# uber/aresdb

Hardware: AMD Instinct MI355X
Metric: rows/sec, 1B-row filter -> group-by-agg (whole job) (higher is better)
Workload: dtype u32 keys / f64 sums; 1 GPU; C3: filter d1<90 -> dims [floor(ts,3600), d1, d2, d3] (4 x uint32) -> SUM(m float32 -> float64) via HashReduce, validity bitmaps with 1% nulls, shard resident in HBM; rows_per_gpu=1000000000, batch_rows=67108864, batches=15, streams_per_query=2, parallelism=1 shard(s), one per GPU

## Files before the change

### aresdb_amd/abi.py

```python
import ctypes as C
import os

_HERE = os.path.dirname(os.path.abspath(__file__))
REPO_ROOT = os.path.dirname(_HERE)
LIB_DIR = os.environ.get("ARES_LIB_DIR") or os.path.join(_HERE, "lib")

AGGR_SUM_UNSIGNED, AGGR_SUM_SIGNED, AGGR_SUM_FLOAT = 1, 2, 3
AGGR_MIN_UNSIGNED, AGGR_MIN_SIGNED, AGGR_MIN_FLOAT = 4, 5, 6
AGGR_MAX_UNSIGNED, AGGR_MAX_SIGNED, AGGR_MAX_FLOAT = 7, 8, 9
AGGR_HLL, AGGR_AVG_FLOAT = 10, 11

(Bool, Int8, Uint8, Int16, Uint16, Int32, Uint32, Float32, Int64, Uint64, Float64, GeoPoint,
 UUID) = range(13)
ConstInt, ConstFloat, ConstGeoPoint, ConstUUID = range(4)
(Negate, Not, BitwiseNot, IsNull, IsNotNull, Noop, GetWeekStart, GetMonthStart, GetQuarterStart,
 GetYearStart, GetDayOfMonth, GetDayOfYear, GetMonthOfYear, GetQuarterOfYear, GetHLLValue,
 ArrayLength) = range(16)
(And, Or, Equal, NotEqual, LessThan, LessThanOrEqual, GreaterThan, GreaterThanOrEqual, Plus, Minus,
 Multiply, Divide, Mod, BitwiseAnd, BitwiseOr, BitwiseXor, Floor, ArrayContains,
 ArrayElementAt) = range(19)
(VectorPartyInput, ScratchSpaceInput, ConstantInput, ForeignColumnInput,
 ArrayVectorPartyInput) = range(5)
ScratchSpaceOutput, MeasureOutput, DimensionOutput = range(3)
NUM_DIM_WIDTH = 5
# ... 277 lines not shown
    def hint_fused_batch(self, query, batch_rows, prev_size, measure_bytes, stream=None, device=0):
        fn = self._algo.AresHintFusedBatch
        fn.argtypes, fn.restype = [C.POINTER(FusedQuery), C.c_int, C.c_int, C.c_int, _S, _I], None
        fn(C.byref(query), int(batch_rows), int(prev_size), int(measure_bytes), stream, device)

    SCAN_AT_FILTER_COUNTERS = ("hints", "scans", "honoured", "declined", "discard_plan", "discard_shape", "discard_touched",
                               "discard_abandoned", "retried", "latched")

    def scan_at_filter_stats(self):
        c = (C.c_ulonglong * len(self.SCAN_AT_FILTER_COUNTERS))()
        self._algo.AresScanAtFilterStats.argtypes, self._algo.AresScanAtFilterStats.restype = [C.POINTER(C.c_ulonglong)], None
        self._algo.AresScanAtFilterStats(c)
        return {k: int(v) for k, v in zip(self.SCAN_AT_FILTER_COUNTERS, c)}

    @property
    def has_fused_select(self):
        return hasattr(self._algo, "AresFusedFilterSelect")

    def fused_filter_select(self, query, batch_rows, limit, out_keys, stream=None, device=0):
        fn = self._algo.AresFusedFilterSelect
        fn.argtypes = [C.POINTER(FusedSelect), C.c_int, C.c_int, DimensionVector, _S, _I]
        fn.restype = CGoCallResHandle
        return _check(fn(C.byref(query), int(batch_rows), int(limit), out_keys, stream, device))

    def select_stats(self):
        c = (C.c_ulonglong * 4)()
        self._algo.AresSelectStats.argtypes, self._algo.AresSelectStats.restype = [C.POINTER(C.c_ulonglong)], None
        self._algo.AresSelectStats(c)
        return {"batches": int(c[0]), "declined": int(c[1]), "tiles": int(c[2]), "rows": int(c[3])}

# ... 128 lines not shown
```

### aresdb_amd/csrc/algo/fused_consumers.hip

```cpp
#include <hip/hip_runtime.h>

#include <cstring>
#include <string>

#include "ares_extensions.h"

#include "deferral.hpp"
#include "hash_reduce_lds.hpp"
#include "sort_reduce_fused.hpp"

namespace ares {

namespace {
struct QueueMatch {
  int prev = 0;
  int dimJob[kFusedDims], measureJob = -1;
  const FilterJournal *journal = nullptr;
  int n0 = 0;
};
bool match_queue(const PendingQueue &pq, const DimensionVector &in, const DimLayoutD &L, int length, QueueMatch *m) {
  const int nd = L.numDims, prev = m->prev = length - pq.n;
  const size_t cap = static_cast<size_t>(in.VectorCapacity);
  if (pq.n <= 0 || prev < 0 || nd < 1 || nd > kFusedDims || in.NumDimsPerDimWidth[0] || in.NumDimsPerDimWidth[1]) return false;
  if (pq.jobs.count != nd && pq.jobs.count != nd + 1) return false;
// ... 131 lines not shown
  *groups = result;
  return true;
}

namespace {
bool hinted_operands(const AresFusedExpr &e, bool compareOnly, int batchRows, hipStream_t stream, FastOperands &f) {
  if (e.arity != 1 && e.arity != 2) return false;
  if (e.lhs.Type != VectorPartyInput || (e.arity == 2 && e.rhs.Type != ConstantInput)) return false;
  if (static_cast<int64_t>(e.lhs.Vector.VP.Length) < batchRows) return false;
  InputVector ins[2] = {e.lhs, e.arity == 2 ? e.rhs : e.lhs};
  EvalParams p;
  CallTemps temps;
  build_params(ins, e.arity, stream, nullptr, nullptr, 0, e.functor, p, temps);
  return p.a.length >= static_cast<uint32_t>(batchRows) && fast_operands(p, f, compareOnly) && f.step == 4;
}
bool hint_fused_batch(int device, hipStream_t stream, const AresFusedQuery &q, int batchRows, int prevSize, int measureBytes) {
  if (!fuse_available() || !row_space_enabled() || !scan_at_filter_enabled()) return false;
  if (q.numDims < 1 || q.numDims > kGenericFusedDims || q.numFilters < 1 || q.numFilters > kExtensionFilters) return false;
  if (batchRows <= 0 || prevSize < 0 || static_cast<int64_t>(batchRows) + prevSize > INT32_MAX) return false;
  if (measureBytes != 4 && measureBytes != 8) return false;
  const int mt = q.measure.outType;
  if (!(mt == Int32 || mt == Uint32 || mt == Float32 || mt == Int64 || mt == Float64) || measureBytes != ((mt == Int64 || mt == Float64) ? 8 : 4))
    return false;
  AggSpec a;
  if (!supported_agg_spec(q.aggFunc, measureBytes, hash_reduce_lds_supported, &a)) return false;
  ScanHint h;
  memset(&h, 0, sizeof(h));
  const int nd = q.numDims;
  h.nd = nd;
  h.batchRows = batchRows;
  h.prevSize = prevSize;
  auto note = [&](const FastOperands &f) {
    column_ranges(f, static_cast<uint32_t>(batchRows), [&](const ByteRange &c) { h.ranges[h.numRanges++] = ScanHint::Range{c.lo, c.hi}; });
  };
  SinkD sink;
  FastOperands f;
  for (int d = 0; d < nd; d++) {
    const int t = q.dims[d].outType;
    if (!(t == Int32 || t == Uint32 || t == Float32) || !hinted_operands(q.dims[d], false, batchRows, stream, f)) return false;
    memset(&sink, 0, sizeof(sink));
    sink.type = SINK_DIM;
// ... 7 lines not shown
  sink.type = SINK_MEASURE;
  sink.dtype = mt;
  sink.width = measureBytes;
  sink.agg = q.aggFunc;
  sink.identity = identity_bits(q.aggFunc, mt);
  if (sink.agg == AGGR_AVG_FLOAT || (measureBytes == 8 && sink.identity != 0)) return false;
  fused_plan_measure(h.plan, nd, f, sink, measureBytes);
  note(f);
  for (int k = 0; k < q.numFilters; k++) {
    if (!hinted_operands(q.filters[k], true, batchRows, stream, f)) return false;
    f.idx = nullptr;
    h.filters[k] = f;
    note(f);
  }
  if (!fused_plan_filters(h.plan, h.filters, static_cast<size_t>(q.numFilters))) return false;
  if (h.plan.numCols > nd + 2 || fused_plan_narrow(h.plan, nd)) return false;
  scan_hint_set(device, stream, h);
  return true;
}
}

namespace {
bool same_vector(const DimensionVector &a, const DimensionVector &b) {
  return a.DimValues == b.DimValues && a.HashValues == b.HashValues && a.IndexVector == b.IndexVector && a.VectorCapacity == b.VectorCapacity &&
         memcmp(a.NumDimsPerDimWidth, b.NumDimsPerDimWidth, sizeof(a.NumDimsPerDimWidth)) == 0;
}
}

static void mark_sort_output(const PendingSort &ps, void *at, size_t bytes, int unit) {
  uint8_t *p = static_cast<uint8_t *>(at);
  retire_fills(range_of(p, bytes), false);
  t_state->fills[p] = PendingFill{ps.stream, bytes, 0, unit, false, ps.keys.IndexVector};
}
// ... 246 lines not shown

void AresHintFusedBatch(const AresFusedQuery *query, int batchRows, int prevSize, int measureBytes, void *cudaStream, int device) {
  bool taken = false;
  try {
    taken = query != nullptr && device >= 0 && device < kMaxDevices &&
            hint_fused_batch(device, reinterpret_cast<hipStream_t>(cudaStream), *query, batchRows, prevSize, measureBytes);
  } catch (std::exception &) {
  }
  if (!taken) scan_ahead_count(kScanAheadDeclined);
}

void AresScanAtFilterStats(unsigned long long *counters) {
  if (counters) scan_ahead_stats(counters);
}

}
```

### aresdb_amd/csrc/algo/hash_reduce_lds.hip

```cpp
#include <hip/hip_runtime.h>

#include <atomic>
#include <functional>
#include <map>
#include <mutex>
#include <string>
#include <unordered_map>

#include <memory>
#include <mutex>
#include <vector>

#include "aggregate.hpp"
#include "common.hpp"
#include "device_model.hpp"
#include "ares_extensions.h"
#include "dim_layout.hpp"
#include "fast_eval.hpp"
#include "hash_reduce_lds.hpp"
#include "hr_kernels.hpp"
#include "hr_rtc.hpp"
#include "sort_reduce_fused.hpp"

namespace ares {
// ... 569 lines not shown
}
static void prepare_direct_scan(Regions &r, const FusedPlanD &plan, int partBits, int64_t rowsA, int batchRows, int prevSize, int streams,
                                int chunkTiles, hipStream_t stream) {
  SlowScope slow("make_regions");
  make_regions(r, partBits, rowsA, batchRows, streams, 4, stream, chunkTiles > 0 ? static_cast<int>(kCompactLineRecords) : 8);
  r.ws.widen = widen_of(plan);
  r.ws.chunkRows = static_cast<uint32_t>(chunkTiles) * 4096u;
  r.ws.rowBase = static_cast<uint32_t>(prevSize);
}

struct ScanStash {
  Regions r;
  FusedPlanD plan;
  int nd, batchRows, prevSize, partBits, chunkTiles, slack;
  RtcKernel lean;
};
namespace {
struct AheadEntry {
  int device;
  hipStream_t stream;
  bool live = false;
  int inits = 0;
  ScanHint hint;
  std::shared_ptr<ScanStash> stash;
  int discardsInARow = 0;
  bool latched = false;
  FusedPlanD latchedShape;
};
std::mutex g_aheadMutex;
std::vector<AheadEntry> g_ahead;
std::atomic<unsigned long long> g_aheadCounters[kScanAheadCounters];

AheadEntry *ahead_find(int device, hipStream_t stream) {
  for (AheadEntry &e : g_ahead)
    if (e.device == device && e.stream == stream) return &e;
  return nullptr;
}
FusedPlanD shape_of(FusedPlanD plan) {
  for (int c = 0; c < kFusedCols; c++) {
    plan.cols[c].vals = nullptr;
    plan.cols[c].nulls = nullptr;
    plan.cols[c].bitOff = 0;
  }
  return plan;
}
void ahead_discarded(AheadEntry &e, int reason) {
  scan_ahead_count(reason);
  if (reason == kScanAheadDiscardRetry) return;
  if (++e.discardsInARow >= 2 && !e.latched) {
    e.latched = true;
    e.latchedShape = shape_of(e.hint.plan);
  }
}
bool ranges_hit(const ScanHint &h, const uint8_t *lo, const uint8_t *hi) {
  for (int k = 0; k < h.numRanges; k++)
    if (h.ranges[k].lo < hi && lo < h.ranges[k].hi) return true;
  return false;
}
}

void scan_ahead_count(int which) { g_aheadCounters[which].fetch_add(1, std::memory_order_relaxed); }
void scan_ahead_stats(unsigned long long *out) {
  for (int k = 0; k < kScanAheadCounters; k++) out[k] = g_aheadCounters[k].load(std::memory_order_relaxed);
}
bool scan_at_filter_enabled() {
  static EnvSwitch<bool> on("ARES_SCAN_AT_FILTER", [](const char *e) { return !(e && e[0] == '0'); });
  return on.get() && grouped_enabled();
}

void scan_hint_set(int device, hipStream_t stream, const ScanHint &hint) {
  std::shared_ptr<ScanStash> old;
  {
    std::lock_guard<std::mutex> lock(g_aheadMutex);
    AheadEntry *e = ahead_find(device, stream);
    if (!e) {
      g_ahead.emplace_back();
      e = &g_ahead.back();
      e->device = device;
      e->stream = stream;
    }
    if (e->stash) ahead_discarded(*e, kScanAheadDiscardAbandoned);
    old.swap(e->stash);
    if (e->latched && fused_plan_equal(shape_of(hint.plan), e->latchedShape, hint.nd)) {
      scan_ahead_count(kScanAheadLatched);
      e->live = false;
      return;
    }
    if (e->latched) {
      e->latched = false;
      e->discardsInARow = 0;
    }
    e->hint = hint;
    e->live = true;
    e->inits = 0;
    scan_ahead_count(kScanAheadHints);
  }
}

void scan_hint_init_index(int device, hipStream_t stream) {
  std::shared_ptr<ScanStash> old;
  std::lock_guard<std::mutex> lock(g_aheadMutex);
  AheadEntry *e = ahead_find(device, stream);
  if (!e) return;
  if (e->stash) ahead_discarded(*e, kScanAheadDiscardAbandoned);
  old.swap(e->stash);
  if (e->live && ++e->inits > 1) e->live = false;
}

bool scan_hint_live(int device, hipStream_t stream, ScanHint *out) {
  std::lock_guard<std::mutex> lock(g_aheadMutex);
  AheadEntry *e = ahead_find(device, stream);
  if (!e || !e->live || e->inits != 1 || e->stash) return false;
  *out = e->hint;
  return true;
}

void scan_stash_put(int device, hipStream_t stream, std::shared_ptr<ScanStash> stash) {
  std::lock_guard<std::mutex> lock(g_aheadMutex);
  AheadEntry *e = ahead_find(device, stream);
  if (!e || !e->live) return;
// ... 17 lines not shown
  if (reason == kScanAheadHonoured) {
    scan_ahead_count(kScanAheadHonoured);
    if (e) e->discardsInARow = 0;
  } else if (e && blame) {
    ahead_discarded(*e, reason);
  } else {
    scan_ahead_count(reason);
  }
}

void scan_ahead_note_touch(int device, const void *ptr, size_t bytes, bool freed) {
  const uint8_t *lo = static_cast<const uint8_t *>(ptr), *hi = lo + (bytes ? bytes : 1);
  std::vector<std::shared_ptr<ScanStash>> dead;
  std::lock_guard<std::mutex> lock(g_aheadMutex);
  for (AheadEntry &e : g_ahead) {
    if (e.device != device || !(e.live || e.stash) || !ranges_hit(e.hint, lo, hi)) continue;
    e.live = false;
    if (e.stash && !freed) {
      scan_ahead_count(kScanAheadDiscardTouched);
      dead.push_back(std::move(e.stash));
      e.stash = nullptr;
    }
  }
}

void scan_ahead_stream_gone(int device, hipStream_t stream) {
  std::shared_ptr<ScanStash> old;
  std::lock_guard<std::mutex> lock(g_aheadMutex);
  for (size_t i = 0; i < g_ahead.size(); i++)
    if (g_ahead[i].device == device && g_ahead[i].stream == stream) {
      if (g_ahead[i].stash) scan_ahead_count(kScanAheadDiscardAbandoned);
      old.swap(g_ahead[i].stash);
      g_ahead[i] = g_ahead.back();
      g_ahead.pop_back();
      return;
    }
}

std::shared_ptr<ScanStash> fused_scan_ahead(int device, const ScanHint &hint, hipStream_t stream, uint32_t *hostCount, int *grid) {
  const FusedPlanD &plan = hint.plan;
  const bool narrow = fused_plan_narrow(plan, hint.nd);
  const int64_t length = static_cast<int64_t>(hint.batchRows) + hint.prevSize;
  if (narrow || hint.batchRows <= 0 || length > INT32_MAX) return nullptr;
  const int partBits = fused_part_bits(length, narrow);
  const ScanChoice choice = choose_scan(device, plan, hint.nd, hint.batchRows, hint.prevSize, partBits, narrow, nullptr);
  if (!choice.wantLean || !choice.lean || !choice.compact) return nullptr;
  auto stash = std::make_shared<ScanStash>();
  stash->plan = plan;
  stash->nd = hint.nd;
  stash->batchRows = hint.batchRows;
  stash->prevSize = hint.prevSize;
  stash->partBits = partBits;
  stash->chunkTiles = choice.chunkTiles;
  stash->slack = record_stream_slack();
  stash->lean = choice.lean;
  const int streams = rtc_scan_grid(hint.batchRows);
  static_assert(kMaxStreams <= kPinnedWords, "one survivor count per workgroup fits the pinned slot");
  prepare_direct_scan(stash->r, plan, partBits, 0, hint.batchRows, hint.prevSize, streams, choice.chunkTiles, stream);
  rtc_scan_launch(choice.lean, RTC_SCAN_COMPACT, plan, static_cast<uint32_t>(hint.prevSize), hint.batchRows, stash->r.ws, stream, hostCount);
  *grid = streams;
  return stash;
}

int fused_hash_reduce_run(int device, const FusedPlanD &plan, int batchRows, const DimensionVector &prevKeys,
                          const uint8_t *prevValues, int prevSize, const DimensionVector &outKeys, uint8_t *outValues,
                          const AggSpec &a, hipStream_t stream, std::shared_ptr<ScanStash> stash) {
  struct Settle {
    std::shared_ptr<ScanStash> &stash;
    int device;
    hipStream_t stream;
    bool taken = false, merged = false;
    void rescanned() {
      if (taken) scan_stash_settled(device, stream, kScanAheadDiscardRetry);
      taken = false;
    }
    ~Settle() {
// ... 345 lines not shown
```

### aresdb_amd/csrc/algo/hash_reduce_lds.hpp

```cpp
#pragma once

#include <hip/hip_runtime.h>

#include <memory>

#include "aggregate.hpp"
#include "ares_algorithm.h"
#include "dim_layout.hpp"
#include "fast_eval.hpp"

namespace ares {

bool hash_reduce_lds_supported(const AggSpec &a);

int hash_reduce_lds(int device, const DimensionVector &inputKeys, const uint8_t *inputValues,
                    const DimensionVector &outputKeys, uint8_t *outputValues, const AggSpec &a, int length,
                    hipStream_t stream);

constexpr int kFusedCols = 10, kFusedFilters = 6, kFusedDims = 8;
constexpr int kGenericFusedDims = 4;
constexpr int kExtensionFilters = 4;
constexpr int kSortVectorValueBytes = 32;
inline bool sort_vector_layout_supported(const uint8_t numDimsPerDimWidth[NUM_DIM_WIDTH]) {
  int nd = 0;
// ... 162 lines not shown
  kScanAheadCounters
};
void scan_ahead_count(int which);
void scan_ahead_stats(unsigned long long *out);
bool scan_at_filter_enabled();
void scan_hint_set(int device, hipStream_t stream, const ScanHint &hint);
void scan_hint_init_index(int device, hipStream_t stream);
bool scan_hint_live(int device, hipStream_t stream, ScanHint *out);
std::shared_ptr<ScanStash> fused_scan_ahead(int device, const ScanHint &hint, hipStream_t stream, uint32_t *hostCount, int *grid);
void scan_stash_put(int device, hipStream_t stream, std::shared_ptr<ScanStash> stash);
std::shared_ptr<ScanStash> scan_stash_take(int device, hipStream_t stream);
void scan_stash_settled(int device, hipStream_t stream, int reason, bool blame = true);
void scan_ahead_note_touch(int device, const void *ptr, size_t bytes, bool freed);
void scan_ahead_stream_gone(int device, hipStream_t stream);

}
```

### aresdb_amd/csrc/algo/transform.hip

```cpp
#include <hip/hip_runtime.h>

#include <algorithm>
#include <cstring>
#include <map>
#include <mutex>

#include "ares_extensions.h"

#include "binding.hpp"
#include "deferral.hpp"
#include "hash_reduce_lds.hpp"
#include "sort_reduce_fused.hpp"

#include "transform_kernels.hpp"

namespace ares {

static void queue_transform(hipStream_t stream, const FastOperands &f, const SinkD &s, int n, uint32_t colRows,
                            std::shared_ptr<StreamBuffer> keep) {
  PendingQueue &q = t_state->pending[stream];
  ByteRange reads[3], writes[2];
  int nr = 0, nw = 0;
  column_ranges(f, colRows, [&](const ByteRange &c) { reads[nr++] = c; });
  if (f.idx) reads[nr++] = range_of(f.idx, 4ull * n);
// ... 487 lines not shown
    count2 += parts[2 * b + 1];
  }
  const PredictedFilter predicted{true, g, static_cast<int>(count2), bits2};
  settle_counted_filter(device, indexVector, generation, static_cast<int>(count), two ? &predicted : nullptr);
  return static_cast<int>(count);
}

int run_filter_scan(int device, hipStream_t stream, FastOperands f, uint32_t *indexVector, uint8_t *pred, int n, uint32_t colRows,
                    bool virtualIdx, const std::shared_ptr<StreamBuffer> &keep) {
  ScanHint hint;
  if (keep || !scan_at_filter_enabled() || !scan_hint_live(device, stream, &hint)) return -1;
  f.idx = nullptr;
  f.pad = 0;
  int grid = 0;
  uint64_t generation = 0;
  {
    DeferLock lock(device);
    auto jr = t_state->journals.find(indexVector);
    if (jr == t_state->journals.end() || !jr->second.valid || jr->second.stream != stream || jr->second.start != 0 ||
        jr->second.n0 != hint.batchRows || jr->second.filters.size() != static_cast<size_t>(hint.plan.numFilters))
      return -1;
    const FilterJournal &j = jr->second;
    for (size_t k = 0; k < j.filters.size(); k++)
      if (!same_filter(j.filters[k], hint.filters[k]) || j.colRows[k] < static_cast<uint32_t>(j.n0)) return -1;
    auto ins = t_state->compactions.find(indexVector);
    if (!row_space_open(jr, ins, stream, n, true)) return -1;
    if (ins != t_state->compactions.end() && ins->second.predicted.valid && same_filter(ins->second.predicted.g, f)) return -1;
    std::shared_ptr<ScanStash> stash = fused_scan_ahead(device, hint, stream, reinterpret_cast<uint32_t *>(pinned_words()), &grid);
    if (!stash) return -1;
    if (ins == t_state->compactions.end()) ins = open_row_space(stream, indexVector, virtualIdx, n);
    PendingCompact &c = ins->second;
    note_filter_shape(t_state->filterHistory[stream], c, f);
    c.predicted = PredictedFilter{};
    generation = book_counted_filter(c, LazyFilter{f, colRows, pred, n, keep}, nullptr, true);
    scan_stash_put(device, stream, std::move(stash));
  }
  hip_check(hipStreamSynchronize(stream), "hipStreamSynchronize");
  const volatile uint32_t *parts = reinterpret_cast<const volatile uint32_t *>(pinned_words());
  uint32_t count = 0;
  for (int b = 0; b < grid; b++) count += parts[b];
  settle_counted_filter(device, indexVector, generation, static_cast<int>(count), nullptr);
  return static_cast<int>(count);
}

bool prepare_filter(int device, hipStream_t stream, const EvalParams &p, uint32_t *indexVector, uint8_t *pred, int n,
                    int numForeignTables, const uint32_t *baseCounts, bool *virtualIdx) {
  bool rowSpace = false;
  *virtualIdx = false;
  FastOperands probe;
  if (!is_wide(p.a.kind) && indexVector != nullptr && numForeignTables == 0 && fast_operands(p, probe, true)) {
    *virtualIdx = virtual_iota(device, indexVector, n, true);
    rowSpace = baseCounts == nullptr && row_space_eligible(device, stream, indexVector, n, p.a.length);
  }
// ... 204 lines not shown
```

### aresdb_amd/csrc/host/abi_library.hpp

```cpp
#pragma once

#include <dlfcn.h>

#include <cstdlib>
#include <cstring>
#include <stdexcept>
#include <string>

#include "ares_driver.h"
#include "ares_extensions.h"
#include "ares_memory.h"

namespace ares_host {

struct AbiError : std::runtime_error {
  explicit AbiError(const std::string &m) : std::runtime_error(m) {}
};

inline intptr_t check(CGoCallResHandle h) {
  if (h.pStrErr) {
    std::string msg(h.pStrErr);
    free(const_cast<char *>(h.pStrErr));
    throw AbiError(msg);
  }
// ... 15 lines not shown

struct AbiLibrary {
  void *algoHandle = nullptr, *memHandle = nullptr;
  decltype(&::InitIndexVector) InitIndexVector;
  decltype(&::HashLookup) HashLookup;
  decltype(&::UnaryTransform) UnaryTransform;
  decltype(&::UnaryFilter) UnaryFilter;
  decltype(&::BinaryTransform) BinaryTransform;
  decltype(&::BinaryFilter) BinaryFilter;
  decltype(&::Sort) Sort;
  decltype(&::Reduce) Reduce;
  decltype(&::HashReduce) HashReduce;
  decltype(&::AresFusedFilterHashReduce) FusedFilterHashReduce = nullptr;
  decltype(&::AresHintFusedBatch) HintFusedBatch = nullptr;
  decltype(&::AresScanAtFilterStats) ScanAtFilterStats = nullptr;
  decltype(&::AresFusedFilterSelect) FusedFilterSelect = nullptr;
  decltype(&::AresFusedFilterJoinSelect) FusedFilterJoinSelect = nullptr;
  decltype(&::AresJoinColumnsRun) JoinColumnsRun = nullptr;
  decltype(&::AresJoinColumnBytes) JoinColumnBytes = nullptr;
  decltype(&::AresGeoShapeColumnRun) GeoShapeColumnRun = nullptr;
  decltype(&::AresGeoShapeColumnBytes) GeoShapeColumnBytes = nullptr;
  decltype(&::AresLocalTimeColumnRun) LocalTimeColumnRun = nullptr;
  decltype(&::Expand) Expand;
  decltype(&::DeviceAllocate) DeviceAllocate;
  decltype(&::DeviceFree) DeviceFree;
  decltype(&::WaitForCudaStream) WaitForCudaStream;
  decltype(&::HyperLogLog) HyperLogLog;
  decltype(&::GeoBatchIntersects) GeoBatchIntersects;
  decltype(&::WriteGeoShapeDim) WriteGeoShapeDim;
  decltype(&::AsyncCopyDeviceToDevice) AsyncCopyDeviceToDevice;
// ... 23 lines not shown
    bind(algoHandle, "HashLookup", HashLookup);
    bind(algoHandle, "UnaryTransform", UnaryTransform);
    bind(algoHandle, "UnaryFilter", UnaryFilter);
    bind(algoHandle, "BinaryTransform", BinaryTransform);
    bind(algoHandle, "BinaryFilter", BinaryFilter);
    bind(algoHandle, "Sort", Sort);
    bind(algoHandle, "Reduce", Reduce);
    bind(algoHandle, "HashReduce", HashReduce);
    bind(algoHandle, "HyperLogLog", HyperLogLog);
    bind(algoHandle, "GeoBatchIntersects", GeoBatchIntersects);
    bind(algoHandle, "WriteGeoShapeDim", WriteGeoShapeDim);
    bind(algoHandle, "Expand", Expand);
    bind(algoHandle, "AresFusedFilterHashReduce", FusedFilterHashReduce, true);
    bind(algoHandle, "AresHintFusedBatch", HintFusedBatch, true);
    bind(algoHandle, "AresScanAtFilterStats", ScanAtFilterStats, true);
    bind(algoHandle, "AresFusedFilterSelect", FusedFilterSelect, true);
    bind(algoHandle, "AresFusedFilterJoinSelect", FusedFilterJoinSelect, true);
    bind(algoHandle, "AresJoinColumnsRun", JoinColumnsRun, true);
    bind(algoHandle, "AresJoinColumnBytes", JoinColumnBytes, true);
    bind(algoHandle, "AresGeoShapeColumnRun", GeoShapeColumnRun, true);
    bind(algoHandle, "AresGeoShapeColumnBytes", GeoShapeColumnBytes, true);
    bind(algoHandle, "AresLocalTimeColumnRun", LocalTimeColumnRun, true);
    bind(memHandle, "DeviceAllocate", DeviceAllocate);
    bind(memHandle, "DeviceFree", DeviceFree);
    bind(memHandle, "WaitForCudaStream", WaitForCudaStream);
    bind(memHandle, "AsyncCopyDeviceToDevice", AsyncCopyDeviceToDevice);
    bind(memHandle, "AsyncCopyDeviceToHost", AsyncCopyDeviceToHost);
    bind(memHandle, "AsyncCopyHostToDevice", AsyncCopyHostToDevice);
    bind(memHandle, "HostAlloc", HostAlloc);
    bind(memHandle, "HostFree", HostFree);
// ... 22 lines not shown
```

### aresdb_amd/csrc/host/batch_executor.cpp

```cpp
#include <algorithm>
#include <cstring>

#include "query.hpp"

using namespace ares_host;

void AresQuery::prepareForFiltering(const VectorPartySlice *cols, int ncols, int n, uint32_t *bc, uint32_t start) {
  columns = cols;
  numColumns = ncols;
  size = n;
  batchRows = n;
  baseCounts = bc;
  startRow = start;
  indexVec = alloc<uint32_t>(static_cast<size_t>(n) * 4);
  predVec = alloc<uint8_t>(static_cast<size_t>(n));
}

void AresQuery::prepareForDimAndMeasureEval() {
  if (resultSize + size <= resultCapacity) return;
  const int oldCapacity = resultCapacity;
  resultCapacity = resultSize + size;
  resultCapacity += resultCapacity / 8;
  const int64_t cap = resultCapacity;
  {
// ... 435 lines not shown
  for (int t : p.dimTypes)
    if (data_type_bytes(t) != 4) return false;
  if (!fusedDims(q->dims, &q->numDims)) return false;
  if (!fusedExpr(p.measureNode, p.measureType, &q->measure)) return false;
  q->aggFunc = static_cast<AggregateFunction>(p.aggFunc);
  return true;
}

void AresQuery::hintBatch() {
  if (!lib->HintFusedBatch || batchPlan->filters.empty()) return;
  Pod<AresFusedQuery> q;
  if (!fusedQuery(&*q)) return;
  lib->HintFusedBatch(&q.get(), batchRows, resultSize, batchPlan->measureBytes(), stream, device);
}

bool AresQuery::runBatchFused(const VectorPartySlice *cols, int ncols, int n) {
  const Plan &p = *batchPlan;
  if (!p.useFusedExtension || fusedDeclined || !lib->FusedFilterHashReduce) return false;
  columns = cols;
  numColumns = ncols;
  Pod<AresFusedQuery> q;
  if (!fusedQuery(&*q)) return false;
  size = n;
  prepareForDimAndMeasureEval();
  calls++;
  CGoCallResHandle h = lib->FusedFilterHashReduce(&q.get(), n, dimensionVector(0), measureVec[0], resultSize,
                                                  dimensionVector(1), measureVec[1], stream, device);
  if (declined(h)) {
    fusedDeclined = true;
    size = 0;
// ... 79 lines not shown
    batchPlan = &rowSpace->plan;
    cols = extendedColumns.data();
    ncols = static_cast<int>(extendedColumns.size());
  }
  if (runBatchFused(cols, ncols, n)) {
    swapStreams();
    return;
  }
  prepareForFiltering(cols, ncols, n, bc, start);
  hintBatch();
  preExec();
  filter();
  join();
  project();
  reduce();
  postExec();
  swapStreams();
}

extern "C" {

void *AresDriverOpen(const char *libalgorithmPath, const char *libmemPath, char *err, int errLen) {
  try {
    return new AbiLibrary(libalgorithmPath, libmemPath);
  } catch (std::exception &e) {
    set_err(err, errLen, e.what());
    return nullptr;
  }
}

// ... 16 lines not shown
  } catch (std::exception &e) {
    set_err(err, errLen, e.what());
    try {
      q->cleanupBeforeAggregation();
    } catch (...) {
    }
    return -1;
  }
}

int AresQueryRunResidentBatches(AresQuery *q, const VectorPartySlice *columns, int numColumns, const int *sizes, int numBatches,
                                char *err, int errLen) {
  for (int b = 0; b < numBatches; b++) {
    q->ownedColumns.clear();
    q->isLastBatch = false;
    const int rc = AresQueryRunBatch(q, columns + static_cast<size_t>(b) * numColumns, numColumns, sizes[b], nullptr, 0, err, errLen);
    if (rc != 0) return rc;
  }
  return 0;
}

int AresQueryResultSize(const AresQuery *q) { return q->plan.isNonAggregation ? q->rowsWritten : q->resultSize; }
int AresQueryDone(const AresQuery *q) { return q->done ? 1 : 0; }
void AresQuerySetMaxBatchSize(AresQuery *q, int rows) { q->maxBatchSize = rows > 0 ? rows : 0; }
int AresQueryResultCapacity(const AresQuery *q) { return q->resultCapacity; }
uint8_t *AresQueryDimensionVector(const AresQuery *q) { return q->dimVec[0]; }
uint8_t *AresQueryMeasureVector(const AresQuery *q) { return q->measureVec[0]; }
long AresQueryNumCalls(const AresQuery *q) { return q->calls; }
long AresQueryNumFusedBatches(const AresQuery *q) { return q->fusedBatches; }
void AresQuerySetLastBatch(AresQuery *q, int isLast) { q->isLastBatch = isLast != 0; }
void AresQuerySetSecondStream(AresQuery *q, void *stream) { q->otherStream = stream; }
// ... 48 lines not shown
```

### aresdb_amd/csrc/host/query.hpp

```cpp
#pragma once

#include <memory>
#include <utility>
#include <vector>

#include "plan.hpp"

namespace ares_host {

struct RowSpace {
  enum Kind { JOIN_COLUMNS, GEO_COLUMN } kind;
  Plan plan;
  std::vector<std::pair<int, int>> leaves;
  int numAdded = 0;
  struct JoinedTable {
    std::vector<int> columns;
    int first = 0;
  };
  std::vector<JoinedTable> tables;
  struct LocalTime {
    int timeColumn;
    int table;
    int zoneColumn;
    int outType;
// ... 25 lines not shown
  uint16_t *hllDimRegIDCount = nullptr;
  size_t hllVectorSize = 0;
  bool isLastBatch = false;
  uint32_t *geoPredicateVec = nullptr;
  int sizeBeforeGeoFilter = 0;
  std::vector<void *> ownedColumns;
  uint64_t *hashVec[2] = {nullptr, nullptr};
  uint32_t *dimIndexVec[2] = {nullptr, nullptr};
  int size = 0;
  uint32_t *indexVec = nullptr;
  uint8_t *predVec = nullptr;
  uint32_t *baseCounts = nullptr;
  uint32_t startRow = 0;
  const VectorPartySlice *columns = nullptr;
  int numColumns = 0;
  std::vector<uint8_t *> stack;
  std::vector<RecordID *> foreignRids;
  std::vector<std::vector<VectorPartySlice>> foreignSliceArrays;
  long calls = 0, fusedBatches = 0;
  bool fusedDeclined = false;
  std::unique_ptr<ares_host::RowSpace> rowSpace;
  bool rowSpaceDeclined = false;
  std::vector<VectorPartySlice> extendedColumns;
  std::vector<void *> joinedOutputs;
  int maxBatchSize = 0;
  int batchRows = 0;
  int rowsWritten = 0;
  bool done = false;
  std::vector<std::vector<uint8_t>> hostSections;

// ... 54 lines not shown
  }
  void runBatch(const VectorPartySlice *cols, int ncols, int n, uint32_t *bc, uint32_t start);

  int recordsNeeded() const { return plan.limit < 0 ? -1 : std::max(plan.limit - rowsWritten, 0); }
  void prepareForDimEval();
  void expandDimensions();
  void projectNonAggr();
  void postExecNonAggr();
  void runBatchNonAggr(const VectorPartySlice *cols, int ncols, int n, uint32_t *bc, uint32_t start);

  bool fusedExpr(int nodeIdx, int outType, AresFusedExpr *e, int *join = nullptr);
  bool fusedFilters(const std::vector<int> &roots, AresFusedExpr *out, int *count, int *joins = nullptr);
  bool fusedDims(AresFusedExpr *out, int *count, int *joins = nullptr);
  bool fusedQuery(AresFusedQuery *q);
  void hintBatch();
  bool runBatchFused(const VectorPartySlice *cols, int ncols, int n);
  bool runBatchFusedSelect(const VectorPartySlice *cols, int ncols, int n);

  void setRowSpace(ares_host::RowSpace::Kind kind, bool on);
  int pruningHints(AresFusedExpr *out);
  bool runJoinColumns(ares_host::RowSpace &rs, int n);
  bool runLocalTimeColumns(ares_host::RowSpace &rs, int n);
  bool runGeoColumn(int n);
  bool resolve(const VectorPartySlice *cols, int ncols, int n);
};
```

### include/ares_extensions.h

```cpp
#ifndef ARES_EXTENSIONS_H_
#define ARES_EXTENSIONS_H_

#include <stddef.h>
#include <stdint.h>

#include "ares_algorithm.h"

#ifdef __cplusplus
extern "C" {
#endif

void AresProfilerEnable(int on);
size_t AresProfilerReport(char *buf, size_t len);

void AresReloadEnv(void);

size_t AresRtcWait(long *counters);

void AresFlushDeferred(int device);
void AresMemSetFlushHook(void (*hook)(int device));

typedef struct {
  void (*flush)(int device);
  void (*on_wait)(int device, void *stream);
// ... 35 lines not shown
typedef struct {
  int numFilters;
  AresFusedExpr filters[4];
  int numDims;
  AresFusedExpr dims[4];
  AresFusedExpr measure;
  enum AggregateFunction aggFunc;
} AresFusedQuery;

CGoCallResHandle AresFusedFilterHashReduce(const AresFusedQuery *query, int batchRows, DimensionVector prevKeys,
                                           uint8_t *prevValues, int prevSize, DimensionVector outKeys,
                                           uint8_t *outValues, void *cudaStream, int device);

void AresHintFusedBatch(const AresFusedQuery *query, int batchRows, int prevSize, int measureBytes, void *cudaStream, int device);
void AresScanAtFilterStats(unsigned long long *counters);

typedef struct {
  int numFilters;
  AresFusedExpr filters[4];
  int numDims;
  AresFusedExpr dims[8];
} AresFusedSelect;

CGoCallResHandle AresFusedFilterSelect(const AresFusedSelect *query, int batchRows, int limit ,
                                       DimensionVector outKeys, void *cudaStream, int device);
void AresSelectStats(unsigned long long *counters);
void AresSelectRunStats(unsigned long long *counters);

typedef struct {
  InputVector key;
// ... 71 lines not shown
```

Measured before the change: 102.1 billion rows/s.

## Launch the filter scan for the next same-stream batch at the end of the current one

```diff
diff --git a/aresdb_amd/abi.py b/aresdb_amd/abi.py
--- a/aresdb_amd/abi.py
+++ b/aresdb_amd/abi.py
@@ -315,6 +315,25 @@
         return {k: int(v) for k, v in zip(self.SCAN_AT_FILTER_COUNTERS, c)}
 
     @property
+    def has_scan_next_batch(self):
+        return hasattr(self._algo, "AresHintNextFusedBatch") and hasattr(self._algo, "AresScanNextBatchStats")
+
+    def hint_next_fused_batch(self, query, batch_rows, expected_prev_size, measure_bytes, stream=None, device=0):
+        fn = self._algo.AresHintNextFusedBatch
+        fn.argtypes, fn.restype = [C.POINTER(FusedQuery), C.c_int, C.c_int, C.c_int, _S, _I], None
+        fn(C.byref(query), int(batch_rows), int(expected_prev_size), int(measure_bytes), stream, device)
+
+    SCAN_NEXT_BATCH_COUNTERS = ("hints", "launched", "adopted", "declined", "drop_other_batch", "drop_shape", "drop_touched",
+                                "drop_abandoned")
+
+    def scan_next_batch_stats(self):
+        c = (C.c_ulonglong * len(self.SCAN_NEXT_BATCH_COUNTERS))()
+        self._algo.AresScanNextBatchStats.argtypes = [C.POINTER(C.c_ulonglong), C.c_int]
+        self._algo.AresScanNextBatchStats.restype = None
+        self._algo.AresScanNextBatchStats(c, len(c))
+        return {k: int(v) for k, v in zip(self.SCAN_NEXT_BATCH_COUNTERS, c)}
+
+    @property
     def has_fused_select(self):
         return hasattr(self._algo, "AresFusedFilterSelect")
 
diff --git a/aresdb_amd/csrc/algo/fused_consumers.hip b/aresdb_amd/csrc/algo/fused_consumers.hip
--- a/aresdb_amd/csrc/algo/fused_consumers.hip
+++ b/aresdb_amd/csrc/algo/fused_consumers.hip
@@ -169,7 +169,7 @@
   build_params(ins, e.arity, stream, nullptr, nullptr, 0, e.functor, p, temps);
   return p.a.length >= static_cast<uint32_t>(batchRows) && fast_operands(p, f, compareOnly) && f.step == 4;
 }
-bool hint_fused_batch(int device, hipStream_t stream, const AresFusedQuery &q, int batchRows, int prevSize, int measureBytes) {
+bool build_scan_hint(hipStream_t stream, const AresFusedQuery &q, int batchRows, int prevSize, int measureBytes, ScanHint &h) {
   if (!fuse_available() || !row_space_enabled() || !scan_at_filter_enabled()) return false;
   if (q.numDims < 1 || q.numDims > kGenericFusedDims || q.numFilters < 1 || q.numFilters > kExtensionFilters) return false;
   if (batchRows <= 0 || prevSize < 0 || static_cast<int64_t>(batchRows) + prevSize > INT32_MAX) return false;
@@ -179,7 +179,6 @@
     return false;
   AggSpec a;
   if (!supported_agg_spec(q.aggFunc, measureBytes, hash_reduce_lds_supported, &a)) return false;
-  ScanHint h;
   memset(&h, 0, sizeof(h));
   const int nd = q.numDims;
   h.nd = nd;
@@ -217,9 +216,18 @@
     note(f);
   }
   if (!fused_plan_filters(h.plan, h.filters, static_cast<size_t>(q.numFilters))) return false;
-  if (h.plan.numCols > nd + 2 || fused_plan_narrow(h.plan, nd)) return false;
+  return h.plan.numCols <= nd + 2 && !fused_plan_narrow(h.plan, nd);
+}
+bool hint_fused_batch(int device, hipStream_t stream, const AresFusedQuery &q, int batchRows, int prevSize, int measureBytes) {
+  ScanHint h;
+  if (!build_scan_hint(stream, q, batchRows, prevSize, measureBytes, h)) return false;
   scan_hint_set(device, stream, h);
   return true;
+}
+bool hint_next_fused_batch(int device, hipStream_t stream, const AresFusedQuery &q, int batchRows, int expectedPrevSize, int measureBytes) {
+  ScanHint h;
+  if (!scan_next_batch_enabled() || !build_scan_hint(stream, q, batchRows, expectedPrevSize, measureBytes, h)) return false;
+  return scan_next_launch(device, stream, h);
 }
 }
 
@@ -496,4 +504,23 @@
   if (counters) scan_ahead_stats(counters);
 }
 
-}
+void AresHintNextFusedBatch(const AresFusedQuery *query, int batchRows, int expectedPrevSize, int measureBytes, void *cudaStream, int device) {
+  bool launched = false;
+  scan_next_count(kScanNextHints);
+  try {
+    if (query != nullptr && device >= 0 && device < kMaxDevices) {
+      hip_check(hipSetDevice(device), "hipSetDevice");
+      CallStreamScope callStreamScope_(cudaStream, __func__);
+      launched = hint_next_fused_batch(device, reinterpret_cast<hipStream_t>(cudaStream), *query, batchRows, expectedPrevSize, measureBytes);
+      if (launched) mem_note_activity();
+    }
+  } catch (std::exception &) {
+  }
+  if (!launched) scan_next_count(kScanNextDeclined);
+}
+
+void AresScanNextBatchStats(unsigned long long *counters, int numCounters) {
+  if (counters && numCounters > 0) scan_next_stats(counters, numCounters);
+}
+
+}
diff --git a/aresdb_amd/csrc/algo/hash_reduce_lds.hip b/aresdb_amd/csrc/algo/hash_reduce_lds.hip
--- a/aresdb_amd/csrc/algo/hash_reduce_lds.hip
+++ b/aresdb_amd/csrc/algo/hash_reduce_lds.hip
@@ -607,6 +607,7 @@
   FusedPlanD plan;
   int nd, batchRows, prevSize, partBits, chunkTiles, slack;
   RtcKernel lean;
+  std::shared_ptr<uint32_t> counts;
 };
 namespace {
 struct AheadEntry {
@@ -619,10 +620,15 @@
   int discardsInARow = 0;
   bool latched = false;
   FusedPlanD latchedShape;
+  bool nextPending = false;
+  bool nextKept = false;
+  ScanHint nextHint;
+  std::shared_ptr<ScanStash> nextStash;
 };
 std::mutex g_aheadMutex;
 std::vector<AheadEntry> g_ahead;
 std::atomic<unsigned long long> g_aheadCounters[kScanAheadCounters];
+std::atomic<unsigned long long> g_nextCounters[kScanNextCounters];
 
 AheadEntry *ahead_find(int device, hipStream_t stream) {
   for (AheadEntry &e : g_ahead)
@@ -650,6 +656,51 @@
     if (h.ranges[k].lo < hi && lo < h.ranges[k].hi) return true;
   return false;
 }
+bool same_batch(const ScanHint &a, const ScanHint &b) {
+  return a.nd == b.nd && a.batchRows == b.batchRows && fused_plan_equal(a.plan, b.plan, a.nd);
+}
+void next_dropped(AheadEntry &e, int reason, std::shared_ptr<ScanStash> *old) {
+  if (e.nextStash) g_nextCounters[reason].fetch_add(1, std::memory_order_relaxed);
+  old->swap(e.nextStash);
+  e.nextStash = nullptr;
+  e.nextPending = false;
+  e.nextKept = false;
+}
+
+struct CountBlock {
+  hipStream_t stream;
+  bool idle;
+  uint32_t *ptr;
+};
+std::mutex g_countMutex;
+std::vector<CountBlock> g_countFree;
+std::map<hipStream_t, uint64_t> g_countEpoch;
+std::shared_ptr<uint32_t> count_block_take(hipStream_t stream) {
+  uint32_t *ptr = nullptr;
+  uint64_t epoch = 0;
+  {
+    std::lock_guard<std::mutex> lock(g_countMutex);
+    epoch = g_countEpoch[stream];
+    for (size_t i = 0; i < g_countFree.size(); i++)
+      if (g_countFree[i].idle || g_countFree[i].stream == stream) {
+        ptr = g_countFree[i].ptr;
+        g_countFree[i] = g_countFree.back();
+        g_countFree.pop_back();
+        break;
+      }
+  }
+  if (!ptr) hip_check(hipHostMalloc(reinterpret_cast<void **>(&ptr), kMaxStreams * sizeof(uint32_t), hipHostMallocPortable | hipHostMallocMapped), "hipHostMalloc");
+  return std::shared_ptr<uint32_t>(ptr, [stream, epoch](uint32_t *p) {
+    std::lock_guard<std::mutex> lock(g_countMutex);
+    g_countFree.push_back(CountBlock{stream, g_countEpoch[stream] != epoch, p});
+  });
+}
+void count_blocks_stream_gone(hipStream_t stream) {
+  std::lock_guard<std::mutex> lock(g_countMutex);
+  g_countEpoch[stream]++;
+  for (CountBlock &b : g_countFree)
+    if (b.stream == stream) b.idle = true;
+}
 }
 
 void scan_ahead_count(int which) { g_aheadCounters[which].fetch_add(1, std::memory_order_relaxed); }
@@ -662,7 +713,7 @@
 }
 
 void scan_hint_set(int device, hipStream_t stream, const ScanHint &hint) {
-  std::shared_ptr<ScanStash> old;
+  std::shared_ptr<ScanStash> old, oldNext;
   {
     std::lock_guard<std::mutex> lock(g_aheadMutex);
     AheadEntry *e = ahead_find(device, stream);
@@ -674,6 +725,10 @@
     }
     if (e->stash) ahead_discarded(*e, kScanAheadDiscardAbandoned);
     old.swap(e->stash);
+    if (e->nextStash || e->nextPending) {
+      e->nextKept = same_batch(e->nextHint, hint);
+      if (!e->nextKept) next_dropped(*e, kScanNextDropOtherBatch, &oldNext);
+    }
     if (e->latched && fused_plan_equal(shape_of(hint.plan), e->latchedShape, hint.nd)) {
       scan_ahead_count(kScanAheadLatched);
       e->live = false;
@@ -691,12 +746,13 @@
 }
 
 void scan_hint_init_index(int device, hipStream_t stream) {
-  std::shared_ptr<ScanStash> old;
+  std::shared_ptr<ScanStash> old, oldNext;
   std::lock_guard<std::mutex> lock(g_aheadMutex);
   AheadEntry *e = ahead_find(device, stream);
   if (!e) return;
   if (e->stash) ahead_discarded(*e, kScanAheadDiscardAbandoned);
   old.swap(e->stash);
+  if ((e->nextStash || e->nextPending) && !(e->nextKept && e->live && e->inits == 0)) next_dropped(*e, kScanNextDropAbandoned, &oldNext);
   if (e->live && ++e->inits > 1) e->live = false;
 }
 
@@ -744,6 +800,10 @@
   std::vector<std::shared_ptr<ScanStash>> dead;
   std::lock_guard<std::mutex> lock(g_aheadMutex);
   for (AheadEntry &e : g_ahead) {
+    if (e.device == device && (e.nextStash || e.nextPending) && ranges_hit(e.nextHint, lo, hi)) {
+      dead.emplace_back();
+      next_dropped(e, kScanNextDropTouched, &dead.back());
+    }
     if (e.device != device || !(e.live || e.stash) || !ranges_hit(e.hint, lo, hi)) continue;
     e.live = false;
     if (e.stash && !freed) {
@@ -755,41 +815,156 @@
 }
 
 void scan_ahead_stream_gone(int device, hipStream_t stream) {
-  std::shared_ptr<ScanStash> old;
-  std::lock_guard<std::mutex> lock(g_aheadMutex);
-  for (size_t i = 0; i < g_ahead.size(); i++)
-    if (g_ahead[i].device == device && g_ahead[i].stream == stream) {
-      if (g_ahead[i].stash) scan_ahead_count(kScanAheadDiscardAbandoned);
-      old.swap(g_ahead[i].stash);
-      g_ahead[i] = g_ahead.back();
-      g_ahead.pop_back();
-      return;
-    }
-}
-
-std::shared_ptr<ScanStash> fused_scan_ahead(int device, const ScanHint &hint, hipStream_t stream, uint32_t *hostCount, int *grid) {
-  const FusedPlanD &plan = hint.plan;
-  const bool narrow = fused_plan_narrow(plan, hint.nd);
+  std::shared_ptr<ScanStash> old, oldNext;
+  {
+    std::lock_guard<std::mutex> lock(g_aheadMutex);
+    for (size_t i = 0; i < g_ahead.size(); i++)
+      if (g_ahead[i].device == device && g_ahead[i].stream == stream) {
+        if (g_ahead[i].stash) scan_ahead_count(kScanAheadDiscardAbandoned);
+        old.swap(g_ahead[i].stash);
+        next_dropped(g_ahead[i], kScanNextDropAbandoned, &oldNext);
+        g_ahead[i] = g_ahead.back();
+        g_ahead.pop_back();
+        break;
+      }
+  }
+  old = nullptr;
+  oldNext = nullptr;
+  count_blocks_stream_gone(stream);
+}
+
+namespace {
+struct AheadChoice {
+  int partBits, chunkTiles, slack, streams;
+  RtcKernel lean;
+};
+bool scan_ahead_choice(int device, const ScanHint &hint, AheadChoice *c) {
+  const bool narrow = fused_plan_narrow(hint.plan, hint.nd);
   const int64_t length = static_cast<int64_t>(hint.batchRows) + hint.prevSize;
-  if (narrow || hint.batchRows <= 0 || length > INT32_MAX) return nullptr;
-  const int partBits = fused_part_bits(length, narrow);
-  const ScanChoice choice = choose_scan(device, plan, hint.nd, hint.batchRows, hint.prevSize, partBits, narrow, nullptr);
-  if (!choice.wantLean || !choice.lean || !choice.compact) return nullptr;
+  if (narrow || hint.batchRows <= 0 || length > INT32_MAX) return false;
+  c->partBits = fused_part_bits(length, narrow);
+  const ScanChoice choice = choose_scan(device, hint.plan, hint.nd, hint.batchRows, hint.prevSize, c->partBits, narrow, nullptr);
+  if (!choice.wantLean || !choice.lean || !choice.compact) return false;
+  c->chunkTiles = choice.chunkTiles;
+  c->slack = record_stream_slack();
+  c->streams = rtc_scan_grid(hint.batchRows);
+  c->lean = choice.lean;
+  return true;
+}
+std::shared_ptr<ScanStash> scan_ahead_launch(const ScanHint &hint, const AheadChoice &c, hipStream_t stream, uint32_t *hostCount) {
   auto stash = std::make_shared<ScanStash>();
-  stash->plan = plan;
+  stash->plan = hint.plan;
   stash->nd = hint.nd;
   stash->batchRows = hint.batchRows;
   stash->prevSize = hint.prevSize;
-  stash->partBits = partBits;
-  stash->chunkTiles = choice.chunkTiles;
-  stash->slack = record_stream_slack();
-  stash->lean = choice.lean;
-  const int streams = rtc_scan_grid(hint.batchRows);
+  stash->partBits = c.partBits;
+  stash->chunkTiles = c.chunkTiles;
+  stash->slack = c.slack;
+  stash->lean = c.lean;
   static_assert(kMaxStreams <= kPinnedWords, "one survivor count per workgroup fits the pinned slot");
-  prepare_direct_scan(stash->r, plan, partBits, 0, hint.batchRows, hint.prevSize, streams, choice.chunkTiles, stream);
-  rtc_scan_launch(choice.lean, RTC_SCAN_COMPACT, plan, static_cast<uint32_t>(hint.prevSize), hint.batchRows, stash->r.ws, stream, hostCount);
-  *grid = streams;
+  prepare_direct_scan(stash->r, hint.plan, c.partBits, 0, hint.batchRows, hint.prevSize, c.streams, c.chunkTiles, stream);
+  rtc_scan_launch(c.lean, RTC_SCAN_COMPACT, hint.plan, static_cast<uint32_t>(hint.prevSize), hint.batchRows, stash->r.ws, stream, hostCount);
   return stash;
+}
+}
+
+std::shared_ptr<ScanStash> fused_scan_ahead(int device, const ScanHint &hint, hipStream_t stream, uint32_t *hostCount, int *grid) {
+  AheadChoice c;
+  if (!scan_ahead_choice(device, hint, &c)) return nullptr;
+  *grid = c.streams;
+  return scan_ahead_launch(hint, c, stream, hostCount);
+}
+
+bool scan_next_batch_enabled() {
+  static EnvSwitch<bool> on("ARES_SCAN_NEXT_BATCH", [](const char *e) { return !(e && e[0] == '0'); });
+  return on.get() && scan_at_filter_enabled();
+}
+void scan_next_count(int which) { g_nextCounters[which].fetch_add(1, std::memory_order_relaxed); }
+void scan_next_stats(unsigned long long *out, int words) {
+  for (int k = 0; k < words; k++) out[k] = k < kScanNextCounters ? g_nextCounters[k].load(std::memory_order_relaxed) : 0ull;
+}
+
+bool scan_next_launch(int device, hipStream_t stream, const ScanHint &hint) {
+  if (!scan_next_batch_enabled()) return false;
+  std::shared_ptr<ScanStash> old;
+  {
+    std::lock_guard<std::mutex> lock(g_aheadMutex);
+    AheadEntry *e = ahead_find(device, stream);
+    if (!e) {
+      g_ahead.emplace_back();
+      e = &g_ahead.back();
+      e->device = device;
+      e->stream = stream;
+    }
+    next_dropped(*e, kScanNextDropAbandoned, &old);
+    if (e->latched && fused_plan_equal(shape_of(hint.plan), e->latchedShape, hint.nd)) return false;
+    e->nextHint = hint;
+    e->nextPending = true;
+  }
+  old = nullptr;
+  std::shared_ptr<ScanStash> stash;
+  bool kept = false;
+  struct Settle {
+    int device;
+    hipStream_t stream;
+    std::shared_ptr<ScanStash> &stash;
+    bool &kept;
+    ~Settle() {
+      std::lock_guard<std::mutex> lock(g_aheadMutex);
+      AheadEntry *e = ahead_find(device, stream);
+      if (!e || !e->nextPending) return;
+      e->nextPending = false;
+      if (stash) {
+        e->nextStash.swap(stash);
+        kept = true;
+      }
+    }
+  };
+  {
+    Settle settle{device, stream, stash, kept};
+    AheadChoice c;
+    if (scan_ahead_choice(device, hint, &c)) {
+      std::shared_ptr<uint32_t> counts = count_block_take(stream);
+      std::shared_ptr<ScanStash> launchedStash = scan_ahead_launch(hint, c, stream, counts.get());
+      launchedStash->counts = std::move(counts);
+      stash = std::move(launchedStash);
+    }
+  }
+  const bool launched = kept || static_cast<bool>(stash);
+  if (launched) scan_next_count(kScanNextLaunched);
+  if (launched && !kept) scan_next_count(kScanNextDropTouched);
+  return launched;
+}
+
+std::shared_ptr<ScanStash> scan_next_adopt(int device, hipStream_t stream, const ScanHint &hint, std::shared_ptr<uint32_t> *counts, int *grid) {
+  std::shared_ptr<ScanStash> st;
+  {
+    std::lock_guard<std::mutex> lock(g_aheadMutex);
+    AheadEntry *e = ahead_find(device, stream);
+    if (!e || !e->nextStash) return nullptr;
+    st.swap(e->nextStash);
+    e->nextKept = false;
+  }
+  int why = -1;
+  AheadChoice c;
+  if (!scan_next_batch_enabled() || st->nd != hint.nd || st->batchRows != hint.batchRows || !fused_plan_equal(st->plan, hint.plan, hint.nd))
+    why = kScanNextDropOtherBatch;
+  else if (!scan_ahead_choice(device, hint, &c) || c.partBits != st->partBits || c.chunkTiles != st->chunkTiles || c.slack != st->slack ||
+           c.lean != st->lean || c.streams != st->r.ws.streams)
+    why = kScanNextDropShape;
+  if (hr_trace_enabled())
+    fprintf(stderr, "scan_next_adopt: %s | rows %d/%d prev %d -> %d partBits %d\n",
+            why < 0 ? "adopted" : why == kScanNextDropOtherBatch ? "dropped (other batch)" : "dropped (shape)", st->batchRows, hint.batchRows,
+            st->prevSize, hint.prevSize, st->partBits);
+  if (why >= 0) {
+    scan_next_count(why);
+    return nullptr;
+  }
+  st->prevSize = hint.prevSize;
+  *counts = st->counts;
+  *grid = c.streams;
+  scan_next_count(kScanNextAdopted);
+  return st;
 }
 
 int fused_hash_reduce_run(int device, const FusedPlanD &plan, int batchRows, const DimensionVector &prevKeys,
diff --git a/aresdb_amd/csrc/algo/hash_reduce_lds.hpp b/aresdb_amd/csrc/algo/hash_reduce_lds.hpp
--- a/aresdb_amd/csrc/algo/hash_reduce_lds.hpp
+++ b/aresdb_amd/csrc/algo/hash_reduce_lds.hpp
@@ -200,4 +200,21 @@
 void scan_ahead_note_touch(int device, const void *ptr, size_t bytes, bool freed);
 void scan_ahead_stream_gone(int device, hipStream_t stream);
 
-}
+enum ScanNextCounter {
+  kScanNextHints,
+  kScanNextLaunched,
+  kScanNextAdopted,
+  kScanNextDeclined,
+  kScanNextDropOtherBatch,
+  kScanNextDropShape,
+  kScanNextDropTouched,
+  kScanNextDropAbandoned,
+  kScanNextCounters
+};
+void scan_next_count(int which);
+void scan_next_stats(unsigned long long *out, int words);
+bool scan_next_batch_enabled();
+bool scan_next_launch(int device, hipStream_t stream, const ScanHint &hint);
+std::shared_ptr<ScanStash> scan_next_adopt(int device, hipStream_t stream, const ScanHint &hint, std::shared_ptr<uint32_t> *counts, int *grid);
+
+}
diff --git a/aresdb_amd/csrc/algo/transform.hip b/aresdb_amd/csrc/algo/transform.hip
--- a/aresdb_amd/csrc/algo/transform.hip
+++ b/aresdb_amd/csrc/algo/transform.hip
@@ -525,6 +525,7 @@
   f.pad = 0;
   int grid = 0;
   uint64_t generation = 0;
+  std::shared_ptr<uint32_t> early;
   {
     DeferLock lock(device);
     auto jr = t_state->journals.find(indexVector);
@@ -537,7 +538,8 @@
     auto ins = t_state->compactions.find(indexVector);
     if (!row_space_open(jr, ins, stream, n, true)) return -1;
     if (ins != t_state->compactions.end() && ins->second.predicted.valid && same_filter(ins->second.predicted.g, f)) return -1;
-    std::shared_ptr<ScanStash> stash = fused_scan_ahead(device, hint, stream, reinterpret_cast<uint32_t *>(pinned_words()), &grid);
+    std::shared_ptr<ScanStash> stash = scan_next_adopt(device, stream, hint, &early, &grid);
+    if (!stash) stash = fused_scan_ahead(device, hint, stream, reinterpret_cast<uint32_t *>(pinned_words()), &grid);
     if (!stash) return -1;
     if (ins == t_state->compactions.end()) ins = open_row_space(stream, indexVector, virtualIdx, n);
     PendingCompact &c = ins->second;
@@ -547,7 +549,7 @@
     scan_stash_put(device, stream, std::move(stash));
   }
   hip_check(hipStreamSynchronize(stream), "hipStreamSynchronize");
-  const volatile uint32_t *parts = reinterpret_cast<const volatile uint32_t *>(pinned_words());
+  const volatile uint32_t *parts = early ? early.get() : reinterpret_cast<const volatile uint32_t *>(pinned_words());
   uint32_t count = 0;
   for (int b = 0; b < grid; b++) count += parts[b];
   settle_counted_filter(device, indexVector, generation, static_cast<int>(count), nullptr);
diff --git a/aresdb_amd/csrc/host/abi_library.hpp b/aresdb_amd/csrc/host/abi_library.hpp
--- a/aresdb_amd/csrc/host/abi_library.hpp
+++ b/aresdb_amd/csrc/host/abi_library.hpp
@@ -53,6 +53,8 @@
   decltype(&::AresFusedFilterHashReduce) FusedFilterHashReduce = nullptr;
   decltype(&::AresHintFusedBatch) HintFusedBatch = nullptr;
   decltype(&::AresScanAtFilterStats) ScanAtFilterStats = nullptr;
+  decltype(&::AresHintNextFusedBatch) HintNextFusedBatch = nullptr;
+  decltype(&::AresScanNextBatchStats) ScanNextBatchStats = nullptr;
   decltype(&::AresFusedFilterSelect) FusedFilterSelect = nullptr;
   decltype(&::AresFusedFilterJoinSelect) FusedFilterJoinSelect = nullptr;
   decltype(&::AresJoinColumnsRun) JoinColumnsRun = nullptr;
@@ -106,6 +108,8 @@
     bind(algoHandle, "AresFusedFilterHashReduce", FusedFilterHashReduce, true);
     bind(algoHandle, "AresHintFusedBatch", HintFusedBatch, true);
     bind(algoHandle, "AresScanAtFilterStats", ScanAtFilterStats, true);
+    bind(algoHandle, "AresHintNextFusedBatch", HintNextFusedBatch, true);
+    bind(algoHandle, "AresScanNextBatchStats", ScanNextBatchStats, true);
     bind(algoHandle, "AresFusedFilterSelect", FusedFilterSelect, true);
     bind(algoHandle, "AresFusedFilterJoinSelect", FusedFilterJoinSelect, true);
     bind(algoHandle, "AresJoinColumnsRun", JoinColumnsRun, true);
diff --git a/aresdb_amd/csrc/host/batch_executor.cpp b/aresdb_amd/csrc/host/batch_executor.cpp
--- a/aresdb_amd/csrc/host/batch_executor.cpp
+++ b/aresdb_amd/csrc/host/batch_executor.cpp
@@ -473,6 +473,17 @@
   lib->HintFusedBatch(&q.get(), batchRows, resultSize, batchPlan->measureBytes(), stream, device);
 }
 
+void AresQuery::hintNextBatch() {
+  if (!aheadColumns || aheadRows <= 0 || resultSize <= 0 || !lib->HintNextFusedBatch) return;
+  if (batchPlan != &plan || batchPlan->filters.empty()) return;
+  const VectorPartySlice *mine = columns;
+  columns = aheadColumns;
+  Pod<AresFusedQuery> q;
+  const bool fits = fusedQuery(&*q);
+  columns = mine;
+  if (fits) lib->HintNextFusedBatch(&q.get(), aheadRows, resultSize, batchPlan->measureBytes(), stream, device);
+}
+
 bool AresQuery::runBatchFused(const VectorPartySlice *cols, int ncols, int n) {
   const Plan &p = *batchPlan;
   if (!p.useFusedExtension || fusedDeclined || !lib->FusedFilterHashReduce) return false;
@@ -582,6 +593,7 @@
   join();
   project();
   reduce();
+  hintNextBatch();
   postExec();
   swapStreams();
 }
@@ -628,7 +640,12 @@
   for (int b = 0; b < numBatches; b++) {
     q->ownedColumns.clear();
     q->isLastBatch = false;
+    const int ahead = b + (q->otherStream ? 2 : 1);
+    q->aheadColumns = ahead < numBatches ? columns + static_cast<size_t>(ahead) * numColumns : nullptr;
+    q->aheadRows = ahead < numBatches ? sizes[ahead] : 0;
     const int rc = AresQueryRunBatch(q, columns + static_cast<size_t>(b) * numColumns, numColumns, sizes[b], nullptr, 0, err, errLen);
+    q->aheadColumns = nullptr;
+    q->aheadRows = 0;
     if (rc != 0) return rc;
   }
   return 0;
diff --git a/aresdb_amd/csrc/host/query.hpp b/aresdb_amd/csrc/host/query.hpp
--- a/aresdb_amd/csrc/host/query.hpp
+++ b/aresdb_amd/csrc/host/query.hpp
@@ -63,6 +63,8 @@
   uint32_t startRow = 0;
   const VectorPartySlice *columns = nullptr;
   int numColumns = 0;
+  const VectorPartySlice *aheadColumns = nullptr;
+  int aheadRows = 0;
   std::vector<uint8_t *> stack;
   std::vector<RecordID *> foreignRids;
   std::vector<std::vector<VectorPartySlice>> foreignSliceArrays;
@@ -147,6 +149,7 @@
   bool fusedDims(AresFusedExpr *out, int *count, int *joins = nullptr);
   bool fusedQuery(AresFusedQuery *q);
   void hintBatch();
+  void hintNextBatch();
   bool runBatchFused(const VectorPartySlice *cols, int ncols, int n);
   bool runBatchFusedSelect(const VectorPartySlice *cols, int ncols, int n);
 
diff --git a/include/ares_extensions.h b/include/ares_extensions.h
--- a/include/ares_extensions.h
+++ b/include/ares_extensions.h
@@ -73,6 +73,9 @@
 
 void AresHintFusedBatch(const AresFusedQuery *query, int batchRows, int prevSize, int measureBytes, void *cudaStream, int device);
 void AresScanAtFilterStats(unsigned long long *counters);
+
+void AresHintNextFusedBatch(const AresFusedQuery *query, int batchRows, int expectedPrevSize, int measureBytes, void *cudaStream, int device);
+void AresScanNextBatchStats(unsigned long long *counters, int numCounters);
 
 typedef struct {
   int numFilters;
```

After: 104.9 billion rows/s (median of 4 runs). 2.7% higher.
